# shiyao-li/NextBestPath

Measured on AMD Instinct MI355X. Metric: exploration steps/s (+ NBP maps/s) at 256x256, higher is better.
Workload: dtype f32

## Files before the change

nextbestpath_amd/csrc/nbp_sim.hip:

```cpp
#include "common.h"
#pragma clang fp contract(off)

namespace {

struct Cam { float R[9]; float T[3]; };
constexpr int MAX_CAMS = 8;
struct CamSet { Cam c[MAX_CAMS]; };

__device__ __forceinline__ void to_view(const float* p, const float* R, const float* T, float* o) {
    o[0] = ((p[0] * R[0] + p[1] * R[3]) + p[2] * R[6]) + T[0];
    o[1] = ((p[0] * R[1] + p[1] * R[4]) + p[2] * R[7]) + T[1];
    o[2] = ((p[0] * R[2] + p[1] * R[5]) + p[2] * R[8]) + T[2];
}

__device__ __forceinline__ void shade_pixel(const float* __restrict__ verts, const int* __restrict__ faces,
                                            const float* __restrict__ vcolors, const Cam& cam, int fi, int row, int col, int H,
                                            int W, float tanh_fov, float ambient, float* rgb3) {
    float v[3][3];
    const int i0 = faces[3 * (size_t)fi], i1 = faces[3 * (size_t)fi + 1], i2 = faces[3 * (size_t)fi + 2];
    to_view(verts + 3 * (size_t)i0, cam.R, cam.T, v[0]);
    to_view(verts + 3 * (size_t)i1, cam.R, cam.T, v[1]);
    to_view(verts + 3 * (size_t)i2, cam.R, cam.T, v[2]);
    float e1[3], e2[3], q[3];
#pragma unroll
// ... 256 lines not shown
        if (in_step) bv.d->n_binned = n < capacity ? n : capacity;
        *done_ticket = 0;
    }
}

constexpr int STEP_BATCH = 12;
struct UnprojItem {
    const float* depth[4]; const unsigned long long* zface[4]; int* blk_count; int* counts; float* cloud;
    long long* cloud_count; long long capacity; float* cloud_rgb; const float* verts; const int* faces;
    const float* vcolors; unsigned seed; Cam cam[4];
};
struct UnprojBatch {
    UnprojItem it[STEP_BATCH]; int ticket_off; unsigned list_off_bytes;
    __device__ int* ticket(int r) const { return it[r].blk_count + ticket_off; }
    __device__ unsigned* list(int r) const { return reinterpret_cast<unsigned*>(reinterpret_cast<char*>(it[r].blk_count) + list_off_bytes); }
};
static_assert(sizeof(UnprojBatch) + 32 <= 4096, "UnprojBatch + the scalar arguments of its kernels must fit 4 KB of kernel arguments");

__global__ __launch_bounds__(256) void unproject_count4_kernel(const float* __restrict__ depth, const unsigned char* __restrict__ mask,
                                                               int HW, int nblk, float fov_range, int* __restrict__ blk_count,
                                                               int* __restrict__ done_ticket) {
    unproject_count4_body(blockIdx.x, blockIdx.y, gridDim.x, gridDim.y, depth, mask, HW, nblk, fov_range, blk_count, done_ticket);
}
__global__ __launch_bounds__(256) void unproject_count4_batch_kernel(UnprojBatch b, int HW, int nblk, float fov_range) {
    const UnprojItem& a = b.it[blockIdx.z];
    unproject_count4_body(blockIdx.x, blockIdx.y, gridDim.x, gridDim.y, a.depth[blockIdx.y] - (size_t)blockIdx.y * HW, nullptr, HW, nblk,
                          fov_range, a.blk_count, b.ticket(blockIdx.z));
}
__global__ __launch_bounds__(256) void unproject_compact4_kernel(const float* __restrict__ depth, const unsigned char* __restrict__ mask,
                                                                 int HW, int nblk, float fov_range, double gather,
                                                                 const int* __restrict__ blk_count, unsigned* __restrict__ list,
                                                                 int* __restrict__ counts) {
    unproject_compact4_body(blockIdx.x, blockIdx.y, gridDim.x, gridDim.y, depth, mask, HW, nblk, fov_range, gather, blk_count, list, counts);
}
__global__ __launch_bounds__(256) void unproject_compact4_batch_kernel(UnprojBatch b, int HW, int nblk, float fov_range, double gather) {
    const UnprojItem& a = b.it[blockIdx.z];
    unproject_compact4_body(blockIdx.x, blockIdx.y, gridDim.x, gridDim.y, a.depth[blockIdx.y] - (size_t)blockIdx.y * HW, nullptr, HW, nblk,
                            fov_range, gather, a.blk_count, b.list(blockIdx.z), a.counts);
}
__global__ __launch_bounds__(256) void unproject_append_kernel(const float* __restrict__ depth, CamSet cams, int H, int W, float tanh_fov,
                                                               unsigned seed, const unsigned* __restrict__ list,
                                                               const int* __restrict__ counts, float* __restrict__ cloud,
                                                               long long* __restrict__ cloud_count, long long capacity, int n_frames,
                                                               int* __restrict__ done_ticket, const float* __restrict__ rgb,
                                                               float* __restrict__ cloud_rgb, const unsigned long long* __restrict__ zface,
                                                               const float* __restrict__ verts, const int* __restrict__ faces,
                                                               const float* __restrict__ vcolors, float ambient, int fence, BinFile bf) {
    unproject_append_body(blockIdx.x, blockIdx.y, gridDim.x, gridDim.y, depth, cams.c, H, W, tanh_fov, seed, list, counts, cloud, cloud_count,
                          capacity, n_frames, done_ticket, rgb, cloud_rgb, zface, verts, faces, vcolors, ambient, fence, bf);
}
__global__ __launch_bounds__(256) void unproject_append_batch_kernel(UnprojBatch b, int H, int W, float tanh_fov, int n_frames, float ambient,
                                                                     int fence) {
    const UnprojItem& a = b.it[blockIdx.z];
    const size_t shift = (size_t)blockIdx.y * H * W;
    unproject_append_body(blockIdx.x, blockIdx.y, gridDim.x, gridDim.y, a.depth[blockIdx.y] - shift, a.cam, H, W, tanh_fov, a.seed,
                          b.list(blockIdx.z), a.counts, a.cloud, a.cloud_count, a.capacity, n_frames, b.ticket(blockIdx.z), nullptr, a.cloud_rgb,
                          a.zface[blockIdx.y] ? a.zface[blockIdx.y] - shift : nullptr, a.verts, a.faces, a.vcolors, ambient, fence);
}

__global__ void cloud_count_update_kernel(const int* __restrict__ counts, int F, long long* __restrict__ cloud_count,
                                          long long capacity) {
    if (blockIdx.x == 0 && threadIdx.x == 0) {
        long long n = *cloud_count;
        for (int f = 0; f < F; ++f) n += counts[2 * f + 1];
        *cloud_count = n < capacity ? n : capacity;
    }
}

constexpr int TILE = 8;
struct FaceRec { float a[3], un[3], q[3], tnum, pad[2]; };

constexpr int COARSE = 8;
constexpr int SEG_DEFAULT = 16384;
constexpr int HITS = 1024;
constexpr unsigned ZBUF_EMPTY = 0x7F7F7F7Fu;

struct BinEntry { int face; unsigned box; };

__device__ __forceinline__ void raster_setup_body(unsigned bx, unsigned by, unsigned gx, unsigned gy, const float* __restrict__ verts, const int* __restrict__ faces,
                                                           int n_faces, const Cam* cams, int H, int W,
                                                           float tanh_fov, float zclip, FaceRec* __restrict__ recs,
                                                           int ctiles_x, int ctiles_y, int* __restrict__ ccount,
                                                           BinEntry* __restrict__ clist, unsigned* __restrict__ zbuf_bits,
                                                           unsigned long long* __restrict__ zface) {
    const int fr = by;
    const int fi = bx * blockDim.x + threadIdx.x;
    if (zface) for (int p = fi; p < H * W; p += gx * blockDim.x) zface[(size_t)fr * H * W + p] = ~0ull;
    else for (int p = fi; p < H * W; p += gx * blockDim.x) zbuf_bits[(size_t)fr * H * W + p] = ZBUF_EMPTY;
    bool have = false;
    int tx0 = 0, tx1 = 0, ty0 = 0, ty1 = 0;
    if (fi < n_faces) {
        const Cam cam = cams[fr];
        float v[3][3];
#pragma unroll
        for (int k = 0; k < 3; ++k) to_view(verts + 3 * (size_t)faces[3 * (size_t)fi + k], cam.R, cam.T, v[k]);
        if (!(v[0][2] <= zclip && v[1][2] <= zclip && v[2][2] <= zclip)) {
            FaceRec r;
            float e1[3], e2[3];
            const float* v0 = v[0];
#pragma unroll
            for (int c = 0; c < 3; ++c) { e1[c] = v[1][c] - v[0][c]; e2[c] = v[2][c] - v[0][c]; }
            r.q[0] = e1[1] * v0[2] - e1[2] * v0[1];
            r.q[1] = e1[2] * v0[0] - e1[0] * v0[2];
            r.q[2] = e1[0] * v0[1] - e1[1] * v0[0];
            r.tnum = (e2[0] * r.q[0] + e2[1] * r.q[1]) + e2[2] * r.q[2];
            r.a[0] = e1[2] * e2[1] - e1[1] * e2[2]; r.a[1] = e1[0] * e2[2] - e1[2] * e2[0]; r.a[2] = e1[1] * e2[0] - e1[0] * e2[1];
            r.un[0] = v0[1] * e2[2] - v0[2] * e2[1]; r.un[1] = v0[2] * e2[0] - v0[0] * e2[2]; r.un[2] = v0[0] * e2[1] - v0[1] * e2[0];
            r.pad[0] = r.pad[1] = 0.f;
            const int s = H < W ? H : W;
            float cmin = 1e30f, cmax = -1e30f, rmin = 1e30f, rmax = -1e30f;
            auto emit = [&](float x, float y, float z) {
                const float nx = x / (z * tanh_fov), ny = y / (z * tanh_fov);
                const float col = ((float)W - (float)s * nx - 1.f) * 0.5f;
                const float row = ((float)H - (float)s * ny - 1.f) * 0.5f;
                cmin = fminf(cmin, col); cmax = fmaxf(cmax, col); rmin = fminf(rmin, row); rmax = fmaxf(rmax, row);
            };
#pragma unroll
            for (int k = 0; k < 3; ++k) {
                const float* a = v[k];
                const float* b = v[(k + 1) % 3];
                const bool ain = a[2] >= zclip, bin_ = b[2] >= zclip;
                if (ain) emit(a[0], a[1], a[2]);
                if (ain != bin_) {
                    const float t = (zclip - a[2]) / (b[2] - a[2]);
                    emit(a[0] + t * (b[0] - a[0]), a[1] + t * (b[1] - a[1]), zclip);
                }
            }
            if (cmax >= cmin) {
                int c0 = (int)floorf(fmaxf(cmin, -1e8f)) - 1, c1 = (int)ceilf(fminf(cmax, 1e8f)) + 1;
                int r0 = (int)floorf(fmaxf(rmin, -1e8f)) - 1, r1 = (int)ceilf(fminf(rmax, 1e8f)) + 1;
                c0 = max(c0, 0); r0 = max(r0, 0); c1 = min(c1, W - 1); r1 = min(r1, H - 1);
                if (c0 <= c1 && r0 <= r1) {
                    recs[(size_t)fr * n_faces + fi] = r;
                    have = true;
                    tx0 = c0 / TILE; tx1 = c1 / TILE; ty0 = r0 / TILE; ty1 = r1 / TILE;
                }
            }
        }
    }
    const int lane = threadIdx.x & 63;
    const unsigned long long lt = (1ull << lane) - 1ull;
    const BinEntry e = {fi, (unsigned)tx0 | ((unsigned)tx1 << 8) | ((unsigned)ty0 << 16) | ((unsigned)ty1 << 24)};
    const int nct = ctiles_x * ctiles_y;
    for (int c0 = 0; c0 < nct; c0 += 64) {
        const int npass = min(64, nct - c0);
        int my_cnt = 0;
        for (int c = 0; c < npass; ++c) {
            const int cx = (c0 + c) % ctiles_x, cy = (c0 + c) / ctiles_x;
            const bool hit = have && tx0 <= cx * COARSE + COARSE - 1 && tx1 >= cx * COARSE && ty0 <= cy * COARSE + COARSE - 1 &&
                             ty1 >= cy * COARSE;
            const int n = __popcll(__ballot(hit));
            if (lane == c) my_cnt = n;
        }
        int my_base = 0;
        if (my_cnt > 0) my_base = atomicAdd(&ccount[fr * nct + c0 + lane], my_cnt);
        for (int c = 0; c < npass; ++c) {
            const int cx = (c0 + c) % ctiles_x, cy = (c0 + c) / ctiles_x;
            const bool hit = have && tx0 <= cx * COARSE + COARSE - 1 && tx1 >= cx * COARSE && ty0 <= cy * COARSE + COARSE - 1 &&
                             ty1 >= cy * COARSE;
            const unsigned long long bal = __ballot(hit);
            const int base = __shfl(my_base, c);
            if (hit) clist[((size_t)fr * nct + c0 + c) * n_faces + base + __popcll(bal & lt)] = e;
        }
    }
}

constexpr int RB = 2;
__device__ __forceinline__ void raster_block_body(unsigned bx, unsigned by, const FaceRec* __restrict__ recs, int n_faces, int H, int W,
                                                  float tanh_fov, float zclip, int tiles_x, int tiles_y, int ctiles_x,
                                                  const int* __restrict__ ccount, const BinEntry* __restrict__ clist,
                                                  unsigned* __restrict__ zbuf_bits, unsigned long long* __restrict__ zface, int SEG) {
    __shared__ BinEntry bhits[HITS];
    __shared__ int nb_sh;
    __shared__ __attribute__((aligned(16))) FaceRec sh[4][64];
    __shared__ int shf[4][64];
    const int fr = by;
    const int blocks_x = (tiles_x + RB - 1) / RB, blocks_y = (tiles_y + RB - 1) / RB;
    const int nblocks = blocks_x * blocks_y;
    const int blk = bx % nblocks, seg = bx / nblocks;
    const int bxx = blk % blocks_x, byy = blk / blocks_x;
    const int nct = ctiles_x * ((tiles_y + COARSE - 1) / COARSE);
    const int ct = ((byy * RB) / COARSE) * ctiles_x + (bxx * RB) / COARSE;
    const int n = ccount[fr * nct + ct];
    const int s0 = seg * SEG;
    if (s0 >= n) return;
    const int s1 = min(n, s0 + SEG);
    const int tid = threadIdx.x, lane = tid & 63, wave = tid >> 6;
    const unsigned long long lt = (1ull << lane) - 1ull;
    const BinEntry* lst = clist + ((size_t)fr * nct + ct) * n_faces;
    const int btx0 = bxx * RB, btx1 = btx0 + RB - 1, bty0 = byy * RB, bty1 = bty0 + RB - 1;
    const int tx = btx0 + (wave & 1), ty = bty0 + (wave >> 1);
    const bool live = tx < tiles_x && ty < tiles_y;
    const int col = tx * TILE + (lane & 7), row = ty * TILE + (lane >> 3);
    const int s = H < W ? H : W;
    const float ndc_x = ((float)W - (2.f * col + 1.f)) / (float)s;
    const float ndc_y = ((float)H - (2.f * row + 1.f)) / (float)s;
    const float dx = ndc_x * tanh_fov, dy = ndc_y * tanh_fov;
    const FaceRec* rb = recs + (size_t)fr * n_faces;
    float zbest = 3.0e38f;
    int fbest = -1;
    const float eps = 1e-6f;
    for (int c0 = s0; c0 < s1; c0 += HITS) {
        const int c1 = min(s1, c0 + HITS);
        if (tid == 0) nb_sh = 0;
        __syncthreads();
        for (int base = c0; base < c1; base += 256) {
            bool in = false;
            BinEntry e = {0, 0u};
            if (base + tid < c1) {
                e = lst[base + tid];
                in = btx1 >= (int)(e.box & 255u) && btx0 <= (int)((e.box >> 8) & 255u) && bty1 >= (int)((e.box >> 16) & 255u) &&
                     bty0 <= (int)(e.box >> 24);
            }
            const unsigned long long bal = __ballot(in);
            int wbase = 0;
            if (lane == 0 && bal) wbase = atomicAdd(&nb_sh, __popcll(bal));
            wbase = __shfl(wbase, 0);
            if (in) bhits[wbase + __popcll(bal & lt)] = e;
        }
        __syncthreads();
        const int nb = nb_sh;
        if (live)
            for (int hb = 0; hb < nb; hb += 64) {
                bool in = false;
                int face = 0;
                if (hb + lane < nb) {
                    const BinEntry e = bhits[hb + lane];
                    face = e.face;
                    in = tx >= (int)(e.box & 255u) && tx <= (int)((e.box >> 8) & 255u) && ty >= (int)((e.box >> 16) & 255u) &&
                         ty <= (int)(e.box >> 24);
                }
                const unsigned long long bal = __ballot(in);
                const int m = __popcll(bal);
                if (in) {
                    const int k = __popcll(bal & lt);
                    sh[wave][k] = rb[face];
                    shf[wave][k] = face;
                }
                __builtin_amdgcn_s_waitcnt(0);
                __builtin_amdgcn_wave_barrier();
                for (int k = 0; k < m; ++k) {
                    const FaceRec& f = sh[wave][k];
                    const float det = (f.a[0] * dx + f.a[1] * dy) + f.a[2];
                    if (fabsf(det) < 1e-12f) continue;
                    const float inv = 1.f / det;
                    const float u = ((f.un[0] * dx + f.un[1] * dy) + f.un[2]) * inv;
                    const float vv = ((dx * f.q[0] + dy * f.q[1]) + f.q[2]) * inv;
                    const float z = f.tnum * inv;
                    if (u >= -eps && vv >= -eps && u + vv <= 1.f + eps && z > zclip) {
                        const int fid = shf[wave][k];
                        if (z < zbest || (z == zbest && fid < fbest)) { zbest = z; fbest = fid; }
                    }
                }
                __builtin_amdgcn_wave_barrier();
            }
        __syncthreads();
    }
    if (live && row < H && col < W && zbest < 1.0e38f) {
        const size_t pix = ((size_t)fr * H + row) * W + col;
        if (zface) atomicMin(&zface[pix], ((unsigned long long)__float_as_uint(zbest) << 32) | (unsigned)fbest);
        else atomicMin(&zbuf_bits[pix], __float_as_uint(zbest));
    }
}

__global__ __launch_bounds__(256) void raster_finalize_kernel(float* __restrict__ zbuf, long long n) {
    for (long long i = (long long)blockIdx.x * blockDim.x + threadIdx.x; i < n; i += (long long)gridDim.x * blockDim.x)
        if (!(zbuf[i] < 1.0e38f)) zbuf[i] = -1.f;
}

__device__ __forceinline__ void raster_shade_body(unsigned bx, unsigned by, unsigned gx, unsigned gy, const unsigned long long* __restrict__ zface,
                                                           const float* __restrict__ verts, const int* __restrict__ faces,
                                                           const float* __restrict__ vcolors, const Cam* cams, int H, int W,
                                                           float tanh_fov, float ambient, float* __restrict__ zbuf_or_null,
                                                           float* __restrict__ rgb_or_null, double* __restrict__ gray_sum) {
    const int fr = by;
    const int p = bx * blockDim.x + threadIdx.x;
    float gray = 0.f;
    if (p < H * W) {
        const size_t pix = (size_t)fr * H * W + p;
        const unsigned long long zf = zface[pix];
        float c[3] = {1.f, 1.f, 1.f};
        if (zbuf_or_null) zbuf_or_null[pix] = zf != ~0ull ? __uint_as_float((unsigned)(zf >> 32)) : -1.f;
        if (rgb_or_null) {
            if (zf != ~0ull) shade_pixel(verts, faces, vcolors, cams[fr], (int)(unsigned)zf, p / W, p % W, H, W, tanh_fov, ambient, c);
            rgb_or_null[3 * pix] = c[0]; rgb_or_null[3 * pix + 1] = c[1]; rgb_or_null[3 * pix + 2] = c[2];
            gray = (0.299f * c[0] + 0.587f * c[1]) + 0.114f * c[2];
        }
    }
    if (!gray_sum) return;
    double gs = (double)gray;
    for (int o = 32; o; o >>= 1) gs += __shfl_xor(gs, o);
    if ((threadIdx.x & 63) == 0) atomicAdd(&gray_sum[fr], gs);
}

struct RasterItem {
    const float* verts; const int* faces; const float* vcolors; FaceRec* recs; int* ccount; BinEntry* clist; float* zbuf;
    unsigned long long* zface; int n_faces; unsigned gx_setup, gx_tile; Cam cam[4];
};
struct RasterBatch { RasterItem it[STEP_BATCH]; };

__global__ __launch_bounds__(256) void raster_setup_kernel(const float* __restrict__ verts, const int* __restrict__ faces, int n_faces,
                                                           CamSet cams, int H, int W, float tanh_fov, float zclip,
                                                           FaceRec* __restrict__ recs, int ctiles_x, int ctiles_y, int* __restrict__ ccount,
                                                           BinEntry* __restrict__ clist, unsigned* __restrict__ zbuf_bits,
                                                           unsigned long long* __restrict__ zface) {
    raster_setup_body(blockIdx.x, blockIdx.y, gridDim.x, gridDim.y, verts, faces, n_faces, cams.c, H, W, tanh_fov, zclip, recs, ctiles_x,
                      ctiles_y, ccount, clist, zbuf_bits, zface);
}
__global__ __launch_bounds__(256) void raster_clear_batch_kernel(RasterBatch b, int n_counters) {
    int* c = b.it[blockIdx.y].ccount;
    for (int i = blockIdx.x * blockDim.x + threadIdx.x; i < n_counters; i += gridDim.x * blockDim.x) c[i] = 0;
}
__global__ __launch_bounds__(256) void raster_setup_batch_kernel(RasterBatch b, int H, int W, float tanh_fov, float zclip, int ctiles_x,
                                                                 int ctiles_y) {
    const RasterItem& a = b.it[blockIdx.z];
    if (blockIdx.x >= a.gx_setup) return;
    raster_setup_body(blockIdx.x, blockIdx.y, a.gx_setup, gridDim.y, a.verts, a.faces, a.n_faces, a.cam, H, W, tanh_fov, zclip, a.recs,
                      ctiles_x, ctiles_y, a.ccount, a.clist, nullptr, a.zface);
}
__global__ __launch_bounds__(256) void raster_tile_kernel(const FaceRec* __restrict__ recs, int n_faces, int H, int W, float tanh_fov,
                                                          float zclip, int tiles_x, int tiles_y, int ctiles_x, int ctiles_y,
                                                          const int* __restrict__ ccount, const BinEntry* __restrict__ clist,
                                                          unsigned* __restrict__ zbuf_bits, unsigned long long* __restrict__ zface, int SEG) {
    raster_block_body(blockIdx.x, blockIdx.y, recs, n_faces, H, W, tanh_fov, zclip, tiles_x, tiles_y, ctiles_x, ccount, clist, zbuf_bits, zface,
                      SEG);
}
__global__ __launch_bounds__(256) void raster_tile_batch_kernel(RasterBatch b, int H, int W, float tanh_fov, float zclip, int tiles_x,
                                                                int tiles_y, int ctiles_x, int ctiles_y, int SEG) {
    const RasterItem& a = b.it[blockIdx.z];
    if (blockIdx.x >= a.gx_tile) return;
    raster_block_body(blockIdx.x, blockIdx.y, a.recs, a.n_faces, H, W, tanh_fov, zclip, tiles_x, tiles_y, ctiles_x, a.ccount, a.clist, nullptr,
                      a.zface, SEG);
}
__global__ __launch_bounds__(256) void raster_shade_kernel(const unsigned long long* __restrict__ zface, const float* __restrict__ verts,
                                                           const int* __restrict__ faces, const float* __restrict__ vcolors, CamSet cams,
                                                           int H, int W, float tanh_fov, float ambient, float* __restrict__ zbuf_or_null,
                                                           float* __restrict__ rgb_or_null, double* __restrict__ gray_sum) {
    raster_shade_body(blockIdx.x, blockIdx.y, gridDim.x, gridDim.y, zface, verts, faces, vcolors, cams.c, H, W, tanh_fov, ambient, zbuf_or_null,
                      rgb_or_null, gray_sum);
}
__global__ __launch_bounds__(256) void raster_depth_batch_kernel(RasterBatch b, int H, int W, float tanh_fov) {
    const RasterItem& a = b.it[blockIdx.z];
    raster_shade_body(blockIdx.x, blockIdx.y, gridDim.x, gridDim.y, a.zface, a.verts, a.faces, a.vcolors, a.cam, H, W, tanh_fov, 0.f, a.zbuf,
                      nullptr, nullptr);
}

__global__ __launch_bounds__(256) void contrast_kernel(float* __restrict__ rgb, int HW3, const double* __restrict__ gray_sum,
                                                       int HW, float factor) {
    const int fr = blockIdx.y;
    const float mean = (float)(gray_sum[fr] / (double)HW);
    for (int i = blockIdx.x * blockDim.x + threadIdx.x; i < HW3; i += gridDim.x * blockDim.x) {
        const float v = factor * rgb[(size_t)fr * HW3 + i] + (1.f - factor) * mean;
        rgb[(size_t)fr * HW3 + i] = fminf(fmaxf(v, 0.f), 1.f);
    }
}

__device__ __forceinline__ float ray_tri(const float* o, const float* d, const float* a, const float* b, const float* c) {
    const float e1[3] = {b[0] - a[0], b[1] - a[1], b[2] - a[2]};
    const float e2[3] = {c[0] - a[0], c[1] - a[1], c[2] - a[2]};
    const float p[3] = {d[1] * e2[2] - d[2] * e2[1], d[2] * e2[0] - d[0] * e2[2], d[0] * e2[1] - d[1] * e2[0]};
    const float det = (e1[0] * p[0] + e1[1] * p[1]) + e1[2] * p[2];
    if (fabsf(det) < 1e-12f) return -1.f;
    const float inv = 1.f / det;
    const float tv[3] = {o[0] - a[0], o[1] - a[1], o[2] - a[2]};
    const float u = ((tv[0] * p[0] + tv[1] * p[1]) + tv[2] * p[2]) * inv;
    if (u < 0.f || u > 1.f) return -1.f;
    const float q[3] = {tv[1] * e1[2] - tv[2] * e1[1], tv[2] * e1[0] - tv[0] * e1[2], tv[0] * e1[1] - tv[1] * e1[0]};
    const float v = ((d[0] * q[0] + d[1] * q[1]) + d[2] * q[2]) * inv;
    if (v < 0.f || u + v > 1.f) return -1.f;
    const float t = ((e2[0] * q[0] + e2[1] * q[1]) + e2[2] * q[2]) * inv;
    return t > 0.f ? t : -1.f;
}

__global__ __launch_bounds__(256) void segments_hit_kernel(const float* __restrict__ verts, const int* __restrict__ faces,
                                                           int n_faces, const float* __restrict__ segs, int* __restrict__ hit) {
    const int e = blockIdx.y;
    const int fi = blockIdx.x * blockDim.x + threadIdx.x;
    if (fi >= n_faces) return;
    const float* sg = segs + 6 * (size_t)e;
    float d[3] = {sg[3] - sg[0], sg[4] - sg[1], sg[5] - sg[2]};
    const float len = sqrtf((d[0] * d[0] + d[1] * d[1]) + d[2] * d[2]);
    if (!(len > 0.f)) return;
    d[0] /= len; d[1] /= len; d[2] /= len;
    const int* f = faces + 3 * (size_t)fi;
    const float t = ray_tri(sg, d, verts + 3 * (size_t)f[0], verts + 3 * (size_t)f[1], verts + 3 * (size_t)f[2]);
    if (t >= 0.f && t < len) atomicOr(&hit[e], 1);
}

__global__ __launch_bounds__(256) void axis_ray_count_kernel(const float* __restrict__ verts, const int* __restrict__ faces,
                                                             int n_faces, const float* __restrict__ pts, int* __restrict__ counts) {
    const int k = blockIdx.y;
    const int fi = blockIdx.x * blockDim.x + threadIdx.x;
    if (fi >= n_faces) return;
    const int* f = faces + 3 * (size_t)fi;
    const float* a = verts + 3 * (size_t)f[0];
    const float* b = verts + 3 * (size_t)f[1];
    const float* c = verts + 3 * (size_t)f[2];
    const float dirs[3][3] = {{0, 1, 0}, {1, 0, 0}, {0, 0, 1}};
#pragma unroll
    for (int ax = 0; ax < 3; ++ax)
        if (ray_tri(pts + 3 * (size_t)k, dirs[ax], a, b, c) >= 0.f) atomicAdd(&counts[3 * k + ax], 1);
}

__device__ __forceinline__ bool point_in_fov(const float* p, const Cam& cam, int H, int W, float tanh_fov, float fov_range,
                                             float* v, float* nx_out, float* ny_out) {
    to_view(p, cam.R, cam.T, v);
    const float cx = -((cam.T[0] * cam.R[0] + cam.T[1] * cam.R[1]) + cam.T[2] * cam.R[2]);
    const float cy = -((cam.T[0] * cam.R[3] + cam.T[1] * cam.R[4]) + cam.T[2] * cam.R[5]);
    const float cz = -((cam.T[0] * cam.R[6] + cam.T[1] * cam.R[7]) + cam.T[2] * cam.R[8]);
    const float dx = p[0] - cx, dy = p[1] - cy, dz = p[2] - cz;
    const float dist = sqrtf((dx * dx + dy * dy) + dz * dz);
    const int s = H < W ? H : W;
    const float nx = v[0] / (v[2] * tanh_fov), ny = v[1] / (v[2] * tanh_fov);
    const float max_x = (float)((double)W / s), min_x = max_x - ((float)(W - 1) / (float)(s - 1)) * 2.f;
    const float max_y = (float)((double)H / s), min_y = max_y - ((float)(H - 1) / (float)(s - 1)) * 2.f;
// ... 217 lines not shown
    int* blk_count = (int*)(((uintptr_t)ws + 255) / 256 * 256);
    unsigned* list = (unsigned*)((char*)blk_count + ((size_t)n_frames * nblk * sizeof(int) + 255) / 256 * 256);
    const CamSet cams = camset_from_host(cams12_host, n_frames);
    const int max_keep = (int)((double)H * W * gathering_factor) + 1;
    dim3 grid((unsigned)nbp_cdiv(max_keep, 256), (unsigned)n_frames);
    int rc;
    const bool fast = (HW & 3) == 0 && ((uintptr_t)depth & 15) == 0 && (!mask_or_null || ((uintptr_t)mask_or_null & 3) == 0);
    NBP_RETURN_IF(bf.store && !fast, NBP_E_SHAPE);
    if (fast) {
        const int nb4 = (int)nbp_cdiv(HW, FAST_CHUNK);
        int* ticket = blk_count + (size_t)n_frames * nb4;
        dim3 g4((unsigned)nb4, (unsigned)n_frames);
        unproject_count4_kernel<<<g4, 256, 0, st>>>(depth, mask_or_null, HW, nb4, fov_range, blk_count, ticket);
        if ((rc = nbp_launch_status())) return rc;
        unproject_compact4_kernel<<<g4, 256, 0, st>>>(depth, mask_or_null, HW, nb4, fov_range, gathering_factor, blk_count, list,
                                                      counts2);
        if ((rc = nbp_launch_status())) return rc;
        if (bf.store && (bf.zero6 || bf.zero1) && grid.x * grid.y < 64u) grid.x = (64u + grid.y - 1) / grid.y;
        unproject_append_kernel<<<grid, 256, 0, st>>>(depth, cams, H, W, tan_half_fov, seed, list, counts2, cloud, cloud_count,
                                                      capacity, n_frames, ticket, rgb_or_null, cloud_rgb_or_null, sh.zface, sh.verts, sh.faces,
                                                      sh.vcolors, sh.ambient, ticket_fence(), bf);
        return nbp_launch_status();
    }
    dim3 gc((unsigned)nblk, (unsigned)n_frames);
    unproject_count_kernel<<<gc, 256, 0, st>>>(depth, mask_or_null, HW, nblk, fov_range, blk_count);
    if ((rc = nbp_launch_status())) return rc;
    unproject_compact_kernel<<<gc, 256, 0, st>>>(depth, mask_or_null, HW, nblk, fov_range, gathering_factor, blk_count,
                                                 list, counts2);
    if ((rc = nbp_launch_status())) return rc;
    unproject_append_kernel<<<grid, 256, 0, st>>>(depth, cams, H, W, tan_half_fov, seed, list, counts2, cloud, cloud_count,
                                                  capacity, n_frames, nullptr, rgb_or_null, cloud_rgb_or_null, sh.zface, sh.verts, sh.faces,
                                                  sh.vcolors, sh.ambient, 0, BinFile{nullptr, nullptr, nullptr, 0});
    if ((rc = nbp_launch_status())) return rc;
    cloud_count_update_kernel<<<1, 64, 0, st>>>(counts2, n_frames, cloud_count, capacity);
    return nbp_launch_status();
}

static size_t raster_ws_bytes(int n_faces, int n_frames, int H, int W, bool rgb) {
    if (n_faces < 1 || n_frames < 1 || H < 1 || W < 1) return 0;
    const size_t nct = (size_t)nbp_cdiv(nbp_cdiv(W, TILE), COARSE) * nbp_cdiv(nbp_cdiv(H, TILE), COARSE) * n_frames;
    size_t b = 256;
    b += ((size_t)n_frames * n_faces * sizeof(FaceRec) + 255) / 256 * 256;
    b += (nct * sizeof(int) + 255) / 256 * 256;
    b += (nct * n_faces * sizeof(BinEntry) + 255) / 256 * 256;
    if (rgb) b += ((size_t)n_frames * H * W * 8 + 255) / 256 * 256 + 256;
    return b + 256;
}

extern "C" size_t nbp_raster_workspace_bytes(int n_faces, int n_frames, int H, int W, int bin_cap) {
    (void)bin_cap;
    return raster_ws_bytes(n_faces, n_frames, H, W, false);
}

extern "C" size_t nbp_raster_rgb_workspace_bytes(int n_faces, int n_frames, int H, int W) {
    return raster_ws_bytes(n_faces, n_frames, H, W, true);
}

static int raster_launch(const float* verts, int n_verts, const int* faces, int n_faces, const float* cams12_host, int n_frames,
                         int H, int W, float tan_half_fov, float z_clip, float* zbuf, const float* vcolors, float ambient,
                         float contrast, float* rgb, void* ws, size_t ws_bytes, void* stream,
                         unsigned long long* zface_out = nullptr) {
    NBP_RETURN_IF(!verts || !faces || !cams12_host || !zbuf || !ws, NBP_E_ARG);
    NBP_RETURN_IF(n_verts < 3 || n_faces < 1 || n_frames < 1 || n_frames > MAX_CAMS || H < 1 || W < 1, NBP_E_ARG);
    const int tiles_x = (int)nbp_cdiv(W, TILE), tiles_y = (int)nbp_cdiv(H, TILE);
    NBP_RETURN_IF(tiles_x > 256 || tiles_y > 256, NBP_E_SHAPE);
    NBP_RETURN_IF(ws_bytes < raster_ws_bytes(n_faces, n_frames, H, W, rgb != nullptr && !zface_out), NBP_E_WS);
    hipStream_t st = (hipStream_t)stream;
    const int ctiles_x = (int)nbp_cdiv(tiles_x, COARSE), ctiles_y = (int)nbp_cdiv(tiles_y, COARSE);
    const size_t nct = (size_t)ctiles_x * ctiles_y * n_frames;
    char* p = (char*)(((uintptr_t)ws + 255) / 256 * 256);
    FaceRec* recs = (FaceRec*)p; p += ((size_t)n_frames * n_faces * sizeof(FaceRec) + 255) / 256 * 256;
    int* ccount = (int*)p; p += (nct * sizeof(int) + 255) / 256 * 256;
    BinEntry* clist = (BinEntry*)p; p += (nct * n_faces * sizeof(BinEntry) + 255) / 256 * 256;
    unsigned long long* zface = nullptr;
    double* gray = nullptr;
    const long long npx = (long long)n_frames * H * W;
    if (zface_out) {
        zface = zface_out;
        gray = (double*)p;
    } else if (rgb) {
        zface = (unsigned long long*)p; p += ((size_t)npx * 8 + 255) / 256 * 256;
        gray = (double*)p;
    }
    hipError_t e = hipMemsetAsync(ccount, 0, nct * sizeof(int), st);
    if (e != hipSuccess) return (int)e;
    dim3 g1((unsigned)nbp_cdiv(n_faces, 256), (unsigned)n_frames);
    raster_setup_kernel<<<g1, 256, 0, st>>>(verts, faces, n_faces, camset_from_host(cams12_host, n_frames), H, W,
                                            tan_half_fov, z_clip, recs, ctiles_x, ctiles_y, ccount, clist, (unsigned*)zbuf, zface);
    int rc = nbp_launch_status();
    if (rc) return rc;
    const bool need_gray = rgb && contrast != 1.f;
    if (need_gray) {
        e = hipMemsetAsync(gray, 0, (size_t)n_frames * sizeof(double), st);
        if (e != hipSuccess) return (int)e;
    }
    constexpr int SEG = SEG_DEFAULT;
    const int nseg = (int)nbp_cdiv(n_faces, SEG);
    dim3 g2((unsigned)((int)nbp_cdiv(tiles_x, RB) * (int)nbp_cdiv(tiles_y, RB) * nseg), (unsigned)n_frames);
    raster_tile_kernel<<<g2, 256, 0, st>>>(recs, n_faces, H, W, tan_half_fov, z_clip, tiles_x, tiles_y, ctiles_x, ctiles_y,
                                          ccount, clist, (unsigned*)zbuf, zface, SEG);
    if ((rc = nbp_launch_status())) return rc;
    if (!zface) {
        raster_finalize_kernel<<<nbp_ew_grid(npx, 256), 256, 0, st>>>(zbuf, npx);
        return nbp_launch_status();
    }
    dim3 g3((unsigned)nbp_cdiv((long long)H * W, 256), (unsigned)n_frames);
    raster_shade_kernel<<<g3, 256, 0, st>>>(zface, verts, faces, vcolors, camset_from_host(cams12_host, n_frames), H, W,
                                            tan_half_fov, ambient, zbuf, rgb, need_gray ? gray : nullptr);
    if ((rc = nbp_launch_status())) return rc;
    if (need_gray) {
        dim3 g4((unsigned)nbp_ew_grid((long long)H * W * 3, 256), (unsigned)n_frames);
        contrast_kernel<<<g4, 256, 0, st>>>(rgb, H * W * 3, gray, H * W, contrast);
        rc = nbp_launch_status();
    }
    return rc;
}

extern "C" int nbp_raster_zbuf_f32(const float* verts, int n_verts, const int* faces, int n_faces, const float* cams12_host,
                                   int n_frames, int H, int W, float tan_half_fov, float z_clip, int bin_cap, float* zbuf,
                                   int* overflow_flag, void* ws, size_t ws_bytes, void* stream) {
    NBP_ENTER();
    (void)bin_cap; (void)overflow_flag;
    return raster_launch(verts, n_verts, faces, n_faces, cams12_host, n_frames, H, W, tan_half_fov, z_clip, zbuf, nullptr, 0.f,
                         1.f, nullptr, ws, ws_bytes, stream);
}

extern "C" int nbp_raster_rgbz_f32(const float* verts, int n_verts, const int* faces, int n_faces, const float* vcolors3,
                                   const float* cams12_host, int n_frames, int H, int W, float tan_half_fov, float z_clip,
                                   float ambient, float contrast_factor, float* zbuf, float* rgb, void* ws, size_t ws_bytes,
                                   void* stream) {
    NBP_ENTER();
    NBP_RETURN_IF(!vcolors3 || !rgb, NBP_E_ARG);
    return raster_launch(verts, n_verts, faces, n_faces, cams12_host, n_frames, H, W, tan_half_fov, z_clip, zbuf, vcolors3,
                         ambient, contrast_factor, rgb, ws, ws_bytes, stream);
}

extern "C" int nbp_raster_zface_f32(const float* verts, int n_verts, const int* faces, int n_faces, const float* cams12_host,
                                    int n_frames, int H, int W, float tan_half_fov, float z_clip, float* zbuf, void* zface,
                                    void* ws, size_t ws_bytes, void* stream) {
    NBP_ENTER();
    NBP_RETURN_IF(!zface, NBP_E_ARG);
    return raster_launch(verts, n_verts, faces, n_faces, cams12_host, n_frames, H, W, tan_half_fov, z_clip, zbuf, nullptr, 0.f,
                         1.f, nullptr, ws, ws_bytes, stream, (unsigned long long*)zface);
}

extern "C" int nbp_unproject_append_shaded_batch_f32(int n, const float* const* depth, const void* const* zface, const float* const* verts,
                                                     const int* const* faces, const float* const* vcolors, const float* cams12_host,
                                                     int n_frames, int H, int W, float tan_half_fov, float fov_range,
                                                     double gathering_factor, const unsigned* seeds, float ambient, int* const* counts2,
                                                     float* const* cloud, float* const* cloud_rgb, long long* const* cloud_count,
                                                     const long long* capacity, void* const* ws, size_t ws_bytes_each, void* stream) {
    NBP_ENTER();
    NBP_RETURN_IF(n < 1 || n > STEP_BATCH || !depth || !cams12_host || !seeds || !counts2 || !cloud || !cloud_count || !capacity || !ws, NBP_E_ARG);
    NBP_RETURN_IF(n_frames < 1 || n_frames > 4 || H < 2 || W < 2 || !(gathering_factor >= 0.0 && gathering_factor <= 1.0), NBP_E_ARG);
    NBP_RETURN_IF(ws_bytes_each < nbp_unproject_workspace_bytes(n_frames, H, W), NBP_E_WS);
    const int HW = H * W;
    NBP_RETURN_IF((HW & 3) != 0, NBP_E_SHAPE);
    hipStream_t st = (hipStream_t)stream;
    const int nblk = (int)nbp_cdiv(HW, COMPACT_CHUNK), nb4 = (int)nbp_cdiv(HW, FAST_CHUNK);
    NBP_RETURN_IF(nblk > 4096, NBP_E_SHAPE);
    UnprojBatch b;
    b.ticket_off = n_frames * nb4;
    b.list_off_bytes = (unsigned)(((size_t)n_frames * nblk * sizeof(int) + 255) / 256 * 256);
    for (int r = 0; r < STEP_BATCH; ++r) {
        const int q = r < n ? r : 0;
        NBP_RETURN_IF(!counts2[q] || !cloud[q] || !cloud_count[q] || capacity[q] < 1 || !ws[q], NBP_E_ARG);
        UnprojItem& a = b.it[r];
        int* blk_count = (int*)(((uintptr_t)ws[q] + 255) / 256 * 256);
        a.blk_count = blk_count;
        a.counts = counts2[q]; a.cloud = cloud[q]; a.cloud_count = cloud_count[q]; a.capacity = capacity[q];
        const bool col = zface && zface[(size_t)q * n_frames] && cloud_rgb && cloud_rgb[q] && verts && faces && vcolors;
        a.cloud_rgb = col ? cloud_rgb[q] : nullptr;
        for (int f = 0; f < 4; ++f) {
            const int g = f < n_frames ? f : 0;
            a.depth[f] = depth[(size_t)q * n_frames + g];
            NBP_RETURN_IF(!a.depth[f] || ((uintptr_t)a.depth[f] & 15) != 0, NBP_E_ARG);
            a.zface[f] = col ? (const unsigned long long*)zface[(size_t)q * n_frames + g] : nullptr;
        }
        a.verts = col ? verts[q] : nullptr; a.faces = col ? faces[q] : nullptr; a.vcolors = col ? vcolors[q] : nullptr;
        a.seed = seeds[q];
        for (int f = 0; f < 4; ++f)
            for (int k = 0; k < 12; ++k) {
                const float v = f < n_frames ? cams12_host[((size_t)q * n_frames + f) * 12 + k] : 0.f;
                if (k < 9) a.cam[f].R[k] = v; else a.cam[f].T[k - 9] = v;
            }
    }
    dim3 g4((unsigned)nb4, (unsigned)n_frames, (unsigned)n);
    unproject_count4_batch_kernel<<<g4, 256, 0, st>>>(b, HW, nb4, fov_range);
    int rc = nbp_launch_status();
    if (rc) return rc;
    unproject_compact4_batch_kernel<<<g4, 256, 0, st>>>(b, HW, nb4, fov_range, gathering_factor);
    if ((rc = nbp_launch_status())) return rc;
    const int max_keep = (int)((double)H * W * gathering_factor) + 1;
    dim3 grid((unsigned)nbp_cdiv(max_keep, 256), (unsigned)n_frames, (unsigned)n);
    unproject_append_batch_kernel<<<grid, 256, 0, st>>>(b, H, W, tan_half_fov, n_frames, ambient, ticket_fence());
    return nbp_launch_status();
}

extern "C" int nbp_raster_zface_batch_f32(int n, const float* const* verts, const int* n_verts, const int* const* faces, const int* n_faces,
                                          const float* cams12_host, int n_frames, int H, int W, float tan_half_fov, float z_clip,
                                          float* const* zbuf, void* const* zface, void* const* ws, const size_t* ws_bytes, void* stream) {
    NBP_ENTER();
    NBP_RETURN_IF(n < 1 || n > STEP_BATCH || !verts || !n_verts || !faces || !n_faces || !cams12_host || !zbuf || !zface || !ws || !ws_bytes,
                  NBP_E_ARG);
    NBP_RETURN_IF(n_frames < 1 || n_frames > 4 || H < 1 || W < 1, NBP_E_ARG);
    const int tiles_x = (int)nbp_cdiv(W, TILE), tiles_y = (int)nbp_cdiv(H, TILE);
    NBP_RETURN_IF(tiles_x > 256 || tiles_y > 256, NBP_E_SHAPE);
    hipStream_t st = (hipStream_t)stream;
    const int ctiles_x = (int)nbp_cdiv(tiles_x, COARSE), ctiles_y = (int)nbp_cdiv(tiles_y, COARSE);
    const size_t nct = (size_t)ctiles_x * ctiles_y * n_frames;
    constexpr int SEG = SEG_DEFAULT;
    RasterBatch b;
    unsigned g_setup = 1, g_tile = 1;
    for (int r = 0; r < STEP_BATCH; ++r) {
        const int q = r < n ? r : 0;
        NBP_RETURN_IF(!verts[q] || !faces[q] || n_verts[q] < 3 || n_faces[q] < 1 || !zbuf[q] || !zface[q] || !ws[q], NBP_E_ARG);
        NBP_RETURN_IF(ws_bytes[q] < raster_ws_bytes(n_faces[q], n_frames, H, W, false), NBP_E_WS);
        RasterItem& a = b.it[r];
        char* p = (char*)(((uintptr_t)ws[q] + 255) / 256 * 256);
        a.recs = (FaceRec*)p; p += ((size_t)n_frames * n_faces[q] * sizeof(FaceRec) + 255) / 256 * 256;
        a.ccount = (int*)p; p += (nct * sizeof(int) + 255) / 256 * 256;
        a.clist = (BinEntry*)p;
        a.verts = verts[q]; a.faces = faces[q]; a.vcolors = nullptr; a.zbuf = zbuf[q]; a.zface = (unsigned long long*)zface[q];
        a.n_faces = n_faces[q];
        a.gx_setup = r < n ? (unsigned)nbp_cdiv(n_faces[q], 256) : 0;
        a.gx_tile = r < n ? (unsigned)((int)nbp_cdiv(tiles_x, RB) * (int)nbp_cdiv(tiles_y, RB) * (int)nbp_cdiv(n_faces[q], SEG)) : 0;
        if (a.gx_setup > g_setup) g_setup = a.gx_setup;
        if (a.gx_tile > g_tile) g_tile = a.gx_tile;
        for (int f = 0; f < 4; ++f)
            for (int k = 0; k < 12; ++k) {
                const float v = f < n_frames ? cams12_host[((size_t)q * n_frames + f) * 12 + k] : 0.f;
                if (k < 9) a.cam[f].R[k] = v; else a.cam[f].T[k - 9] = v;
            }
    }
    raster_clear_batch_kernel<<<dim3(1, (unsigned)n), 256, 0, st>>>(b, (int)nct);
    int rc = nbp_launch_status();
    if (rc) return rc;
    raster_setup_batch_kernel<<<dim3(g_setup, (unsigned)n_frames, (unsigned)n), 256, 0, st>>>(b, H, W, tan_half_fov, z_clip, ctiles_x, ctiles_y);
    if ((rc = nbp_launch_status())) return rc;
    raster_tile_batch_kernel<<<dim3(g_tile, (unsigned)n_frames, (unsigned)n), 256, 0, st>>>(b, H, W, tan_half_fov, z_clip, tiles_x, tiles_y,
                                                                                          ctiles_x, ctiles_y, SEG);
    if ((rc = nbp_launch_status())) return rc;
    raster_depth_batch_kernel<<<dim3((unsigned)nbp_cdiv((long long)H * W, 256), (unsigned)n_frames, (unsigned)n), 256, 0, st>>>(b, H, W,
                                                                                                                          tan_half_fov);
    return nbp_launch_status();
}

extern "C" int nbp_shade_image_f32(const void* zface, const float* verts, const int* faces, const float* vcolors3,
                                   const float* cams12_host, int n_frames, int H, int W, float tan_half_fov, float ambient,
                                   float contrast_factor, float* rgb, void* stream) {
    NBP_ENTER();
    NBP_RETURN_IF(!zface || !verts || !faces || !vcolors3 || !cams12_host || !rgb, NBP_E_ARG);
    NBP_RETURN_IF(n_frames < 1 || n_frames > MAX_CAMS || H < 1 || W < 1, NBP_E_ARG);
    NBP_RETURN_IF(contrast_factor != 1.f, NBP_E_SHAPE);
    dim3 g3((unsigned)nbp_cdiv((long long)H * W, 256), (unsigned)n_frames);
    raster_shade_kernel<<<g3, 256, 0, (hipStream_t)stream>>>((const unsigned long long*)zface, verts, faces, vcolors3,
                                                             camset_from_host(cams12_host, n_frames), H, W, tan_half_fov,
                                                             ambient, nullptr, rgb, nullptr);
    return nbp_launch_status();
}

extern "C" int nbp_segments_hit_mesh_f32(const float* verts, const int* faces, int n_faces, const float* segs6, int n_segs,
                                         int* hit, void* stream) {
    NBP_ENTER();
    NBP_RETURN_IF(!verts || !faces || !segs6 || !hit || n_faces < 1 || n_segs < 1 || n_segs > 65535, NBP_E_ARG);
    hipStream_t st = (hipStream_t)stream;
    hipError_t e = hipMemsetAsync(hit, 0, (size_t)n_segs * sizeof(int), st);
    if (e != hipSuccess) return (int)e;
    dim3 g((unsigned)nbp_cdiv(n_faces, 256), (unsigned)n_segs);
    segments_hit_kernel<<<g, 256, 0, st>>>(verts, faces, n_faces, segs6, hit);
    return nbp_launch_status();
}

extern "C" int nbp_axis_ray_counts_f32(const float* verts, const int* faces, int n_faces, const float* pts3, int n_pts,
                                       int* counts3, void* stream) {
    NBP_ENTER();
    NBP_RETURN_IF(!verts || !faces || !pts3 || !counts3 || n_faces < 1 || n_pts < 1 || n_pts > 65535, NBP_E_ARG);
    hipStream_t st = (hipStream_t)stream;
    hipError_t e = hipMemsetAsync(counts3, 0, (size_t)n_pts * 3 * sizeof(int), st);
    if (e != hipSuccess) return (int)e;
    dim3 g((unsigned)nbp_cdiv(n_faces, 256), (unsigned)n_pts);
    axis_ray_count_kernel<<<g, 256, 0, st>>>(verts, faces, n_faces, pts3, counts3);
    return nbp_launch_status();
}

extern "C" int nbp_carve_update_f32(const float* proxy_pts3, int P, const float* depth, const unsigned char* mask_or_null,
                                    const float* cam12_host, int H, int W, float tan_half_fov, float zfar, float fov_range,
                                    float tol, float score_threshold, float* n_inside, float* n_behind, float* occ,
                                    float* out_of_field, void* stream) {
    NBP_ENTER();
    NBP_RETURN_IF(!proxy_pts3 || !depth || !cam12_host || !n_inside || !n_behind || !occ || !out_of_field, NBP_E_ARG);
    NBP_RETURN_IF(P < 1 || H < 2 || W < 2, NBP_E_ARG);
    Cam cam;
    for (int k = 0; k < 9; ++k) cam.R[k] = cam12_host[k];
    for (int k = 0; k < 3; ++k) cam.T[k] = cam12_host[9 + k];
    carve_update_kernel<<<(unsigned)nbp_cdiv(P, 256), 256, 0, (hipStream_t)stream>>>(
        proxy_pts3, P, depth, mask_or_null, cam, H, W, tan_half_fov, zfar, fov_range, tol, score_threshold, n_inside,
        n_behind, occ, out_of_field, nullptr, 0.f, ViewArgs{}, nullptr, nullptr);
    return nbp_launch_status();
}

static int view_args_from_host(const float* x_view_host, int n_view, int n_elev, int n_azim, ViewArgs* va) {
    NBP_RETURN_IF(!x_view_host || n_view < 1 || n_view > MAX_CAMS || n_elev < 1 || n_azim < 1 || (long long)n_elev * n_azim > 4096, NBP_E_ARG);
    for (int k = 0; k < 3 * MAX_CAMS; ++k) va->x[k] = k < 3 * n_view ? x_view_host[k] : 0.f;
    va->n_view = n_view; va->n_elev = n_elev; va->n_azim = n_azim;
    const double es = 3.14159265358979323846 / (n_elev + 1), as = 2.0 * 3.14159265358979323846 / n_azim;
    va->elev_step = (float)es; va->azim_step = (float)as; va->half_e = (float)(es / 2.0); va->half_a = (float)(as / 2.0);
    return 0;
}

extern "C" int nbp_view_state_update_f32(const float* pts3, int P, const unsigned char* mask_or_null, const float* sd_or_null,
                                         float distance_to_surface, const float* x_view_host, int n_view, int n_elev, int n_azim,
                                         float* view_states, void* stream) {
    NBP_ENTER();
    NBP_RETURN_IF(!pts3 || !view_states || P < 1, NBP_E_ARG);
    ViewArgs va;
    const int rc = view_args_from_host(x_view_host, n_view, n_elev, n_azim, &va);
    if (rc) return rc;
    view_state_kernel<<<(unsigned)nbp_cdiv(P, 256), 256, 0, (hipStream_t)stream>>>(pts3, P, mask_or_null, sd_or_null, distance_to_surface,
                                                                                 va, view_states);
    return nbp_launch_status();
}
// ... 207 lines not shown
```

Baseline: 2302.

## Write depth directly from tile owner when one face segment covers all

```diff
diff --git a/nextbestpath_amd/csrc/nbp_sim.hip b/nextbestpath_amd/csrc/nbp_sim.hip
--- a/nextbestpath_amd/csrc/nbp_sim.hip
+++ b/nextbestpath_amd/csrc/nbp_sim.hip
@@ -362,11 +362,13 @@
                                                            float tanh_fov, float zclip, FaceRec* __restrict__ recs,
                                                            int ctiles_x, int ctiles_y, int* __restrict__ ccount,
                                                            BinEntry* __restrict__ clist, unsigned* __restrict__ zbuf_bits,
-                                                           unsigned long long* __restrict__ zface) {
+                                                           unsigned long long* __restrict__ zface, bool clear) {
     const int fr = by;
     const int fi = bx * blockDim.x + threadIdx.x;
-    if (zface) for (int p = fi; p < H * W; p += gx * blockDim.x) zface[(size_t)fr * H * W + p] = ~0ull;
-    else for (int p = fi; p < H * W; p += gx * blockDim.x) zbuf_bits[(size_t)fr * H * W + p] = ZBUF_EMPTY;
+    if (clear) {
+        if (zface) for (int p = fi; p < H * W; p += gx * blockDim.x) zface[(size_t)fr * H * W + p] = ~0ull;
+        else for (int p = fi; p < H * W; p += gx * blockDim.x) zbuf_bits[(size_t)fr * H * W + p] = ZBUF_EMPTY;
+    }
     bool have = false;
     int tx0 = 0, tx1 = 0, ty0 = 0, ty1 = 0;
     if (fi < n_faces) {
@@ -446,6 +448,7 @@
 }
 
 constexpr int RB = 2;
+template <bool OWNER>
 __device__ __forceinline__ void raster_block_body(unsigned bx, unsigned by, const FaceRec* __restrict__ recs, int n_faces, int H, int W,
                                                   float tanh_fov, float zclip, int tiles_x, int tiles_y, int ctiles_x,
                                                   const int* __restrict__ ccount, const BinEntry* __restrict__ clist,
@@ -463,7 +466,7 @@
     const int ct = ((byy * RB) / COARSE) * ctiles_x + (bxx * RB) / COARSE;
     const int n = ccount[fr * nct + ct];
     const int s0 = seg * SEG;
-    if (s0 >= n) return;
+    if (!OWNER && s0 >= n) return;
     const int s1 = min(n, s0 + SEG);
     const int tid = threadIdx.x, lane = tid & 63, wave = tid >> 6;
     const unsigned long long lt = (1ull << lane) - 1ull;
@@ -476,6 +479,7 @@
     const float ndc_x = ((float)W - (2.f * col + 1.f)) / (float)s;
     const float ndc_y = ((float)H - (2.f * row + 1.f)) / (float)s;
     const float dx = ndc_x * tanh_fov, dy = ndc_y * tanh_fov;
+    const bool stored = live && row < H && col < W;
     const FaceRec* rb = recs + (size_t)fr * n_faces;
     float zbest = 3.0e38f;
     int fbest = -1;
@@ -536,7 +540,14 @@
             }
         __syncthreads();
     }
-    if (live && row < H && col < W && zbest < 1.0e38f) {
+    if (OWNER) {
+        if (stored) {
+            const size_t pix = ((size_t)fr * H + row) * W + col;
+            const bool hit = zbest < 1.0e38f;
+            if (zface) zface[pix] = hit ? ((unsigned long long)__float_as_uint(zbest) << 32) | (unsigned)fbest : ~0ull;
+            if (zbuf_bits) zbuf_bits[pix] = __float_as_uint(hit ? zbest : -1.f);
+        }
+    } else if (stored && zbest < 1.0e38f) {
         const size_t pix = ((size_t)fr * H + row) * W + col;
         if (zface) atomicMin(&zface[pix], ((unsigned long long)__float_as_uint(zbest) << 32) | (unsigned)fbest);
         else atomicMin(&zbuf_bits[pix], __float_as_uint(zbest));
@@ -583,34 +594,49 @@
                                                            CamSet cams, int H, int W, float tanh_fov, float zclip,
                                                            FaceRec* __restrict__ recs, int ctiles_x, int ctiles_y, int* __restrict__ ccount,
                                                            BinEntry* __restrict__ clist, unsigned* __restrict__ zbuf_bits,
-                                                           unsigned long long* __restrict__ zface) {
+                                                           unsigned long long* __restrict__ zface, bool clear) {
     raster_setup_body(blockIdx.x, blockIdx.y, gridDim.x, gridDim.y, verts, faces, n_faces, cams.c, H, W, tanh_fov, zclip, recs, ctiles_x,
-                      ctiles_y, ccount, clist, zbuf_bits, zface);
+                      ctiles_y, ccount, clist, zbuf_bits, zface, clear);
 }
 __global__ __launch_bounds__(256) void raster_clear_batch_kernel(RasterBatch b, int n_counters) {
     int* c = b.it[blockIdx.y].ccount;
     for (int i = blockIdx.x * blockDim.x + threadIdx.x; i < n_counters; i += gridDim.x * blockDim.x) c[i] = 0;
 }
 __global__ __launch_bounds__(256) void raster_setup_batch_kernel(RasterBatch b, int H, int W, float tanh_fov, float zclip, int ctiles_x,
-                                                                 int ctiles_y) {
+                                                                 int ctiles_y, bool clear) {
     const RasterItem& a = b.it[blockIdx.z];
     if (blockIdx.x >= a.gx_setup) return;
     raster_setup_body(blockIdx.x, blockIdx.y, a.gx_setup, gridDim.y, a.verts, a.faces, a.n_faces, a.cam, H, W, tanh_fov, zclip, a.recs,
-                      ctiles_x, ctiles_y, a.ccount, a.clist, nullptr, a.zface);
+                      ctiles_x, ctiles_y, a.ccount, a.clist, nullptr, a.zface, clear);
 }
 __global__ __launch_bounds__(256) void raster_tile_kernel(const FaceRec* __restrict__ recs, int n_faces, int H, int W, float tanh_fov,
                                                           float zclip, int tiles_x, int tiles_y, int ctiles_x, int ctiles_y,
                                                           const int* __restrict__ ccount, const BinEntry* __restrict__ clist,
                                                           unsigned* __restrict__ zbuf_bits, unsigned long long* __restrict__ zface, int SEG) {
-    raster_block_body(blockIdx.x, blockIdx.y, recs, n_faces, H, W, tanh_fov, zclip, tiles_x, tiles_y, ctiles_x, ccount, clist, zbuf_bits, zface,
-                      SEG);
+    raster_block_body<false>(blockIdx.x, blockIdx.y, recs, n_faces, H, W, tanh_fov, zclip, tiles_x, tiles_y, ctiles_x, ccount, clist, zbuf_bits,
+                             zface, SEG);
+}
+__global__ __launch_bounds__(256) void raster_tile_owner_kernel(const FaceRec* __restrict__ recs, int n_faces, int H, int W, float tanh_fov,
+                                                                float zclip, int tiles_x, int tiles_y, int ctiles_x, int ctiles_y,
+                                                                const int* __restrict__ ccount, const BinEntry* __restrict__ clist,
+                                                                unsigned* __restrict__ zbuf_bits, unsigned long long* __restrict__ zface,
+                                                                int SEG) {
+    raster_block_body<true>(blockIdx.x, blockIdx.y, recs, n_faces, H, W, tanh_fov, zclip, tiles_x, tiles_y, ctiles_x, ccount, clist, zbuf_bits,
+                            zface, SEG);
+}
+__global__ __launch_bounds__(256) void raster_tile_owner_batch_kernel(RasterBatch b, int H, int W, float tanh_fov, float zclip, int tiles_x,
+                                                                      int tiles_y, int ctiles_x, int ctiles_y, int SEG) {
+    const RasterItem& a = b.it[blockIdx.z];
+    if (blockIdx.x >= a.gx_tile) return;
+    raster_block_body<true>(blockIdx.x, blockIdx.y, a.recs, a.n_faces, H, W, tanh_fov, zclip, tiles_x, tiles_y, ctiles_x, a.ccount, a.clist,
+                            (unsigned*)a.zbuf, a.zface, SEG);
 }
 __global__ __launch_bounds__(256) void raster_tile_batch_kernel(RasterBatch b, int H, int W, float tanh_fov, float zclip, int tiles_x,
                                                                 int tiles_y, int ctiles_x, int ctiles_y, int SEG) {
     const RasterItem& a = b.it[blockIdx.z];
     if (blockIdx.x >= a.gx_tile) return;
-    raster_block_body(blockIdx.x, blockIdx.y, a.recs, a.n_faces, H, W, tanh_fov, zclip, tiles_x, tiles_y, ctiles_x, a.ccount, a.clist, nullptr,
-                      a.zface, SEG);
+    raster_block_body<false>(blockIdx.x, blockIdx.y, a.recs, a.n_faces, H, W, tanh_fov, zclip, tiles_x, tiles_y, ctiles_x, a.ccount, a.clist,
+                             nullptr, a.zface, SEG);
 }
 __global__ __launch_bounds__(256) void raster_shade_kernel(const unsigned long long* __restrict__ zface, const float* __restrict__ verts,
                                                            const int* __restrict__ faces, const float* __restrict__ vcolors, CamSet cams,
@@ -994,11 +1020,14 @@
         zface = (unsigned long long*)p; p += ((size_t)npx * 8 + 255) / 256 * 256;
         gray = (double*)p;
     }
+    constexpr int SEG = SEG_DEFAULT;
+    const int nseg = (int)nbp_cdiv(n_faces, SEG);
+    const bool owner = nseg == 1;
     hipError_t e = hipMemsetAsync(ccount, 0, nct * sizeof(int), st);
     if (e != hipSuccess) return (int)e;
     dim3 g1((unsigned)nbp_cdiv(n_faces, 256), (unsigned)n_frames);
     raster_setup_kernel<<<g1, 256, 0, st>>>(verts, faces, n_faces, camset_from_host(cams12_host, n_frames), H, W,
-                                            tan_half_fov, z_clip, recs, ctiles_x, ctiles_y, ccount, clist, (unsigned*)zbuf, zface);
+                                            tan_half_fov, z_clip, recs, ctiles_x, ctiles_y, ccount, clist, (unsigned*)zbuf, zface, !owner);
     int rc = nbp_launch_status();
     if (rc) return rc;
     const bool need_gray = rgb && contrast != 1.f;
@@ -1006,19 +1035,23 @@
         e = hipMemsetAsync(gray, 0, (size_t)n_frames * sizeof(double), st);
         if (e != hipSuccess) return (int)e;
     }
-    constexpr int SEG = SEG_DEFAULT;
-    const int nseg = (int)nbp_cdiv(n_faces, SEG);
     dim3 g2((unsigned)((int)nbp_cdiv(tiles_x, RB) * (int)nbp_cdiv(tiles_y, RB) * nseg), (unsigned)n_frames);
-    raster_tile_kernel<<<g2, 256, 0, st>>>(recs, n_faces, H, W, tan_half_fov, z_clip, tiles_x, tiles_y, ctiles_x, ctiles_y,
-                                          ccount, clist, (unsigned*)zbuf, zface, SEG);
+    if (owner)
+        raster_tile_owner_kernel<<<g2, 256, 0, st>>>(recs, n_faces, H, W, tan_half_fov, z_clip, tiles_x, tiles_y, ctiles_x, ctiles_y,
+                                                    ccount, clist, (unsigned*)zbuf, zface, SEG);
+    else
+        raster_tile_kernel<<<g2, 256, 0, st>>>(recs, n_faces, H, W, tan_half_fov, z_clip, tiles_x, tiles_y, ctiles_x, ctiles_y,
+                                              ccount, clist, (unsigned*)zbuf, zface, SEG);
     if ((rc = nbp_launch_status())) return rc;
     if (!zface) {
+        if (owner) return 0;
         raster_finalize_kernel<<<nbp_ew_grid(npx, 256), 256, 0, st>>>(zbuf, npx);
         return nbp_launch_status();
     }
+    if (owner && !rgb) return 0;
     dim3 g3((unsigned)nbp_cdiv((long long)H * W, 256), (unsigned)n_frames);
     raster_shade_kernel<<<g3, 256, 0, st>>>(zface, verts, faces, vcolors, camset_from_host(cams12_host, n_frames), H, W,
-                                            tan_half_fov, ambient, zbuf, rgb, need_gray ? gray : nullptr);
+                                            tan_half_fov, ambient, owner ? nullptr : zbuf, rgb, need_gray ? gray : nullptr);
     if ((rc = nbp_launch_status())) return rc;
     if (need_gray) {
         dim3 g4((unsigned)nbp_ew_grid((long long)H * W * 3, 256), (unsigned)n_frames);
@@ -1124,6 +1157,7 @@
     constexpr int SEG = SEG_DEFAULT;
     RasterBatch b;
     unsigned g_setup = 1, g_tile = 1;
+    bool owner = true;
     for (int r = 0; r < STEP_BATCH; ++r) {
         const int q = r < n ? r : 0;
         NBP_RETURN_IF(!verts[q] || !faces[q] || n_verts[q] < 3 || n_faces[q] < 1 || !zbuf[q] || !zface[q] || !ws[q], NBP_E_ARG);
@@ -1135,6 +1169,7 @@
         a.clist = (BinEntry*)p;
         a.verts = verts[q]; a.faces = faces[q]; a.vcolors = nullptr; a.zbuf = zbuf[q]; a.zface = (unsigned long long*)zface[q];
         a.n_faces = n_faces[q];
+        owner = owner && n_faces[q] <= SEG;
         a.gx_setup = r < n ? (unsigned)nbp_cdiv(n_faces[q], 256) : 0;
         a.gx_tile = r < n ? (unsigned)((int)nbp_cdiv(tiles_x, RB) * (int)nbp_cdiv(tiles_y, RB) * (int)nbp_cdiv(n_faces[q], SEG)) : 0;
         if (a.gx_setup > g_setup) g_setup = a.gx_setup;
@@ -1148,8 +1183,14 @@
     raster_clear_batch_kernel<<<dim3(1, (unsigned)n), 256, 0, st>>>(b, (int)nct);
     int rc = nbp_launch_status();
     if (rc) return rc;
-    raster_setup_batch_kernel<<<dim3(g_setup, (unsigned)n_frames, (unsigned)n), 256, 0, st>>>(b, H, W, tan_half_fov, z_clip, ctiles_x, ctiles_y);
+    raster_setup_batch_kernel<<<dim3(g_setup, (unsigned)n_frames, (unsigned)n), 256, 0, st>>>(b, H, W, tan_half_fov, z_clip, ctiles_x, ctiles_y,
+                                                                                            !owner);
     if ((rc = nbp_launch_status())) return rc;
+    if (owner) {
+        raster_tile_owner_batch_kernel<<<dim3(g_tile, (unsigned)n_frames, (unsigned)n), 256, 0, st>>>(b, H, W, tan_half_fov, z_clip, tiles_x,
+                                                                                                    tiles_y, ctiles_x, ctiles_y, SEG);
+        return nbp_launch_status();
+    }
     raster_tile_batch_kernel<<<dim3(g_tile, (unsigned)n_frames, (unsigned)n), 256, 0, st>>>(b, H, W, tan_half_fov, z_clip, tiles_x, tiles_y,
                                                                                           ctiles_x, ctiles_y, SEG);
     if ((rc = nbp_launch_status())) return rc;
```

Result: slower. 2263 (-1.7%).
